# DredderGun/accbpg_and_fw

Hardware: AMD Instinct MI355X
Metric: D-opt iters/sec (m=2048,n=32768) (higher is better)
Workload: dtype f64; 1 GPU; D_opt_design(2048,32768) abpg_gain gamma=2 fp64, one independent instance per GPU; instances=1, instances_per_gpu=1, seeds=1..1, window=transient: iterations 5..161 from x0 = 1/n, linear_gram=False

## Files before the change

### accbpg_and_fw_amd/csrc/capi.hip

```cpp
#include <stdarg.h>
#include <string.h>
#include <stdlib.h>
#include <algorithm>

#include "internal.h"
#include "reduce.hpp"

namespace accbpg {

static thread_local char g_err[512] = "";

void set_last_error(const char* fmt, ...) {
    va_list ap;
    va_start(ap, fmt);
    vsnprintf(g_err, sizeof(g_err), fmt, ap);
    va_end(ap);
}

void note_tiles_fallback(const char* where) {
    static bool said = false;
    if (said) return;
    said = true;
    fprintf(stderr, "libaccbpg_hip: %s: the one-launch Cholesky abandoned a wait (another process on this GPU, or fewer "
                    "workgroups resident than the occupancy query promised); this handle factors with one launch per block "
// ... 462 lines not shown

extern "C" int accbpg_test_gemm(const double* A_dev, int64_t lda, const double* B_dev, int64_t ldb, double* C_dev,
                                int64_t ldc, int64_t M, int64_t N, int64_t K, int b_kmajor, double alpha,
                                double beta, int config, void* stream) {
    if (!A_dev || !B_dev || !C_dev || M <= 0 || N <= 0 || K <= 0) return ACCBPG_ERR_ARG;
    return launch_test_gemm(A_dev, lda, B_dev, ldb, C_dev, ldc, M, N, K, b_kmajor, alpha, beta, config,
                            (hipStream_t)stream);
}

extern "C" int accbpg_dopt_factor_in_small_launches(accbpg_dopt* h, int on) {
    if (!h || on < 0 || on > 2) return ACCBPG_ERR_ARG;
    const int64_t T = (h->m + NB - 1) / NB;
    value_forget(h);
    h->chol_tiles_off = on == 1 || (on == 2 && T * (T + 1) / 2 >= h->num_cu);
    return ACCBPG_OK;
}

extern "C" int accbpg_debug_plan_flags(int flags) {
    set_plan_flags(flags);
    return ACCBPG_OK;
}

extern "C" int accbpg_debug_chol_variant(accbpg_dopt* h, int bits) {
    if (!h) return ACCBPG_ERR_ARG;
    value_forget(h);
    h->chol_dbg = bits & 63;
    h->chol_tiles_off = (bits & 64) != 0;
    if (bits & 2048) h->chol_tiles_off = true;
    h->chol_stall_test = (bits & 128) ? 1 : 0;
    h->chol_spin_limit = (bits & 128) ? 200000 : 20000000;
    h->kern_variant = (bits >> 30) & 3;
    if (bits & 256) h->use_glds = false;
    if (bits & 512) h->use_glds = true;
    if (bits & 2048) {
        h->chol_two_level_T = (bits >> 12) & 0xfff;
        if ((bits >> 24) & 0x3f) h->chol_nk = (bits >> 24) & 0x3f;
    }
    return ACCBPG_OK;
}

extern "C" int accbpg_debug_chol_trace(accbpg_dopt* h, const double* gram_dev, int with_inverse, int64_t* stamps_host) {
    if (!h || !gram_dev || !stamps_host) return ACCBPG_ERR_ARG;
    if (!chol_tiles_usable(h)) {
        set_last_error("accbpg_debug_chol_trace: the one-launch Cholesky is not in use for this handle");
        return ACCBPG_ERR_ARG;
    }
    const int T = (int)((h->m + NB - 1) / NB);
    const size_t bytes = sizeof(long long) * (size_t)T * 32;
    if (!h->chol_trace) ACC_HIP(hipMalloc(&h->chol_trace, bytes));
    ACC_HIP(hipMemsetAsync(h->chol_trace, 0, bytes, h->stream));
    int rc = launch_cholesky(h, h->Lbuf, with_inverse ? h->Wbuf : nullptr, nullptr, gram_dev);
    if (rc == ACCBPG_OK) {
        hipError_t e = hipMemcpyAsync(stamps_host, h->chol_trace, bytes, hipMemcpyDeviceToHost, h->stream);
        if (e == hipSuccess) e = hipStreamSynchronize(h->stream);
        if (e != hipSuccess) rc = ACCBPG_ERR_HIP;
    }
    hipFree(h->chol_trace);
    h->chol_trace = nullptr;
    return rc;
}

extern "C" int accbpg_debug_gram_variant(accbpg_dopt* h, const double* x_dev, int variant, int iters, double* ms_host) {
    if (!h || !x_dev || !ms_host || iters <= 0) return ACCBPG_ERR_ARG;
    value_forget(h);
    return debug_gram_variant(h, x_dev, variant, iters, ms_host);
}
// ... 7 lines not shown
```

### accbpg_and_fw_amd/csrc/dopt_kernels.hip

```cpp
#include <mutex>
#include <unordered_map>
#include <type_traits>

#include "internal.h"
#include "mfma_tile.hpp"

namespace accbpg {

struct GramSeg {
    int64_t row0, col0, kb, ke;
    bool dual, whole;
};
constexpr int GRAM_RMAX = 4;
template <class T>
__device__ __forceinline__ GramSeg gram_segment(const TileRC* __restrict__ tiles, int64_t kiters, int64_t it,
                                                int64_t it1) {
    const int e = (int)(it / kiters);
    const int64_t off = it - (int64_t)e * kiters;
    const TileRC tr = tiles[e];
    GramSeg g;
    if (tr.d1 < 0) {
        g.row0 = (int64_t)tr.rb * T::BM; g.col0 = (int64_t)tr.cb * T::BN;
        g.kb = off; g.ke = min(kiters, off + (it1 - it));
        g.dual = false;
// ... 747 lines not shown
    }
    __syncthreads();
    for (int c = threadIdx.x; c < T::BN; c += NTHREADS) {
        double s = 0.0;
#pragma unroll
        for (int w = 0; w < T::WAVES_M; ++w) s += red[w * T::BN + c];
        if (col0 + c < n) out[col0 + c] = sign * s;
    }
}

template <class T, int CV = 0>
__device__ __forceinline__ void colnorm_glds_body(
    const double* __restrict__ W, int64_t ldw, const double* __restrict__ V, int64_t ldv, int64_t m, int64_t n,
    double* __restrict__ out, double sign) {
    if constexpr (CV == COLNORM_CV) colnorm_phases_body<T>(W, ldw, V, ldv, m, n, out, sign);
    else colnorm_restart_body<T, CV>(W, ldw, V, ldv, m, n, out, sign);
}

template <class T, int CV = 0>
__global__ __launch_bounds__(NTHREADS, 1) void colnorm_glds_kernel(
    const double* __restrict__ W, int64_t ldw, const double* __restrict__ V, int64_t ldv, int64_t m, int64_t n,
    double* __restrict__ out, double sign) {
    colnorm_glds_body<T, CV>(W, ldw, V, ldv, m, n, out, sign);
}
template <class T>
__global__ __launch_bounds__(NTHREADS, 1) void colnorm_glds_batch_kernel(
    const BatchInst* __restrict__ bt, BatchAct act, int64_t ldw, int64_t ldv, int64_t m, int64_t n,
    double* __restrict__ outbase, int64_t ldo, double sign) {
    const int inst = act.idx[blockIdx.y];
    const BatchInst bi = bt[inst];
    colnorm_glds_body<T, COLNORM_CV>(bi.Wbuf, ldw, bi.V, ldv, m, n, outbase + (int64_t)inst * ldo, sign);
}

template <class T>
__device__ __forceinline__ void gemm_ops_body(const GemmOp op) {
    extern __shared__ __attribute__((aligned(16))) double lds[];
    const int64_t row0 = (int64_t)blockIdx.y * T::BM, col0 = (int64_t)blockIdx.x * T::BN;
    if (row0 >= op.M || col0 >= op.N) return;
    if (op.lower_only && col0 > row0 + T::BM - 1) return;
    const bool va = ((reinterpret_cast<uintptr_t>(op.A) & 15) == 0) && ((op.lda & 1) == 0);
    const bool vb = ((reinterpret_cast<uintptr_t>(op.B) & 15) == 0) && ((op.ldb & 1) == 0);
    T t;
    t.zero();
    int64_t ksteps = (op.K + BK - 1) / BK;
    int64_t ks0 = 0;
    if (op.tri & 1) ks0 = max((int64_t)0, col0 - op.koff) / BK;
    if (op.tri & 2) ksteps = min(ksteps, max((int64_t)0, row0 + T::BM - op.koff + BK - 1) / BK);
    if (ks0 >= ksteps) {
        t.store_C(op.C, op.ldc, row0, col0, op.M, op.N, op.alpha, op.beta, op.lower_only != 0);
        return;
    }
    auto gload = [&](int64_t ks) {
        t.gload_A(op.A, op.lda, row0, op.M, ks * BK, op.K, va);
        if constexpr (T::BKM) t.gload_B_km(op.B, op.ldb, col0, op.N, ks * BK, op.K, vb);
        else t.gload_B_kc(op.B, op.ldb, col0, op.N, ks * BK, op.K, vb);
    };
    gload(ks0);
    t.sstore(lds);
    __syncthreads();
    int cur = 0;
    for (int64_t ks = ks0; ks < ksteps; ++ks) {
        const bool more = ks + 1 < ksteps;
        if (more) gload(ks + 1);
        t.compute(lds + cur * T::STAGE_ELEMS);
        if (more) t.sstore(lds + (cur ^ 1) * T::STAGE_ELEMS);
        __syncthreads();
        cur ^= 1;
    }
    t.store_C(op.C, op.ldc, row0, col0, op.M, op.N, op.alpha, op.beta, op.lower_only != 0);
}

template <class T>
__global__ __launch_bounds__(NTHREADS, 2) void gemm_ops_kernel(const GemmOp* __restrict__ ops) {
    gemm_ops_body<T>(ops[blockIdx.z]);
}
template <class T>
__global__ __launch_bounds__(NTHREADS, 2) void gemm_ops_batch_kernel(const GemmOp* __restrict__ ops, int per_inst, int begin,
                                                                    int count, BatchAct act) {
    const int a = blockIdx.z / count, o = blockIdx.z - a * count;
    gemm_ops_body<T>(ops[(int64_t)act.idx[a] * per_inst + begin + o]);
}

__device__ __forceinline__ void gemm_reduce_body(const RedOp r) {
    const int64_t total = (int64_t)r.M * r.N;
    const int64_t stride = (int64_t)gridDim.x * 256 * 2;
    for (int64_t e = 2 * ((int64_t)blockIdx.x * 256 + threadIdx.x); e < total; e += stride) {
        double2 acc = *reinterpret_cast<const double2*>(r.P + e);
        for (int p = 1; p < r.ns; ++p) {
            const double2 v = *reinterpret_cast<const double2*>(r.P + (int64_t)p * total + e);
            acc.x += v.x;
            acc.y += v.y;
        }
        const int64_t row = e / r.N, col = e - row * r.N;
        *reinterpret_cast<double2*>(r.C + row * r.ldc + col) = acc;
    }
}
__global__ __launch_bounds__(256) void gemm_reduce_kernel(const RedOp* __restrict__ reds) { gemm_reduce_body(reds[blockIdx.y]); }
__global__ __launch_bounds__(256) void gemm_reduce_batch_kernel(const RedOp* __restrict__ reds, int per_inst, int begin, int count,
                                                               BatchAct act) {
    const int a = blockIdx.y / count, o = blockIdx.y - a * count;
    gemm_reduce_body(reds[(int64_t)act.idx[a] * per_inst + begin + o]);
}

template <class T>
__global__ __launch_bounds__(NTHREADS, 1) void gemm_big_kernel(GemmOp op) {
    extern __shared__ __attribute__((aligned(16))) double lds[];
    const int64_t row0 = (int64_t)blockIdx.y * T::BM, col0 = (int64_t)blockIdx.x * T::BN;
    if (row0 >= op.M || col0 >= op.N) return;
    const bool va = ((reinterpret_cast<uintptr_t>(op.A) & 15) == 0) && ((op.lda & 1) == 0);
    const bool vb = ((reinterpret_cast<uintptr_t>(op.B) & 15) == 0) && ((op.ldb & 1) == 0);
    T t;
    t.zero();
    const int64_t ksteps = (op.K + BK - 1) / BK;
// ... 1404 lines not shown
    if (T <= CT_TMAX) {
        std::vector<CholJob> jobs;
        for (int d2 = 0; d2 < T; ++d2) jobs.push_back(CholJob{d2, d2});
        for (int j = 0; j < T; ++j)
            for (int i = j + 2; i < T; ++i) jobs.push_back(CholJob{i, j});
        ACC_TRY(set_lds(chol_tiles_kernel, CT_LDS_BYTES));
        int per_cu = 0;
        ACC_HIP(hipOccupancyMaxActiveBlocksPerMultiprocessor(&per_cu, chol_tiles_kernel, NTHREADS, CT_LDS_BYTES));
        h->chol_tiles_grid = (int)jobs.size();
        h->chol_slots = std::min(per_cu, 2) * h->num_cu;
        h->chol_tiles_ok = per_cu >= 1 && (int64_t)jobs.size() <= (int64_t)h->chol_slots;
        if (h->chol_tiles_ok) {
            ACC_HIP(hipMalloc(&h->chol_jobs, sizeof(CholJob) * jobs.size()));
            ACC_HIP(hipMemcpy(h->chol_jobs, jobs.data(), sizeof(CholJob) * jobs.size(), hipMemcpyHostToDevice));
            ACC_HIP(hipMalloc(&h->chol_ready, sizeof(int) * (size_t)(T * T + 5 * T)));
            ACC_HIP(hipMemset(h->chol_ready, 0, sizeof(int) * (size_t)(T * T + 5 * T)));
            ACC_HIP(hipMalloc(&h->chol_hand, sizeof(double) * (size_t)T * NB * NB));
            ACC_HIP(hipMalloc(&h->chol_aux, sizeof(double) * (size_t)T * CT_AUX));
            ACC_HIP(hipMalloc(&h->Gbuf, sizeof(double) * (size_t)m * m));
            ACC_HIP(hipMemset(h->Gbuf, 0, sizeof(double) * (size_t)m * m));
        }
    }

    ACC_TRY(set_lds(gram_streamk_kernel<TileBig<false, true>>, TileBig<false>::LDS_BYTES));
    ACC_TRY(set_lds(gram_streamk_kernel<TileBig<false, false>>, TileBig<false>::LDS_BYTES));
    ACC_TRY(set_lds(gram_streamk_kernel<TileSmall<false, true>>, TileSmall<false>::LDS_BYTES));
    ACC_TRY(set_lds(gram_streamk_kernel<TileSmall<false, false>>, TileSmall<false>::LDS_BYTES));
    ACC_TRY(set_lds(colnorm_kernel<TileBig<true, true>>, TileBig<true>::LDS_BYTES));
    ACC_TRY(set_lds(colnorm_kernel<TileBig<true, false>>, TileBig<true>::LDS_BYTES));
    ACC_TRY(set_lds(colnorm_kernel<TileSmall<true, true>>, TileSmall<true>::LDS_BYTES));
    ACC_TRY(set_lds(colnorm_kernel<TileSmall<true, false>>, TileSmall<true>::LDS_BYTES));
    ACC_TRY(set_lds(gemm_ops_kernel<TileSmall<true>>, TileSmall<true>::LDS_BYTES));
    ACC_TRY(set_lds(gemm_ops_kernel<TileSmall<false>>, TileSmall<false>::LDS_BYTES));
    ACC_TRY(set_lds(chol_step_kernel, CHOL_LDS_BYTES));
    ACC_TRY(set_lds(chol_syrk_kernel, SYRK_LDS_BYTES));
    ACC_TRY(set_lds(gemm_big_kernel<TileBig<true>>, TileBig<true>::LDS_BYTES));
    ACC_TRY(set_lds(gemm_big_kernel<TileBig<false>>, TileBig<false>::LDS_BYTES));
    return ACCBPG_OK;
}

template <class T>
static int gram_launch_t(accbpg_dopt* h, const double* x, double* gram) {
    if constexpr (!T::EDGE && T::BM == 256) {
        if (h->use_glds || h->has_duals) {
            const int64_t nc = h->gram_chunks > 1 ? h->gram_nc : h->n;
            for (int c = 0; c < h->gram_chunks; ++c) {
                const double* Vc = h->Vblk ? h->Vblk + (int64_t)c * h->m * nc : h->V + (int64_t)c * nc;
                const int64_t ldc = h->Vblk ? nc : h->ldv;
                const double* xc = x + (int64_t)c * nc;
                const double beta = c == 0 ? 0.0 : 1.0;
                const int all_slabs = h->gram_chunks > 1 ? 1 : 0;
                prof_begin(h, PROF_GRAM);
#define ACC_GRAM_ARGS Vc, ldc, h->m, nc, xc, h->tiles, h->wg_ranges, h->kiters, h->gram_nslot, h->slabs, gram, h->m, all_slabs
                if (h->kern_variant == 1)
                    ACC_LAUNCH_LDS((gram_streamk_glds_kernel<T, GRAM_GV ^ 128>), h->gram_grid, NTHREADS, T::G_LDS_BYTES, h->stream, ACC_GRAM_ARGS);
                else if (h->kern_variant == 3)
                    ACC_LAUNCH_LDS((gram_streamk_glds_kernel<T, 0>), h->gram_grid, NTHREADS, T::G_LDS_BYTES, h->stream, ACC_GRAM_ARGS);
                else if (h->kern_variant == 2)
                    ACC_LAUNCH_LDS((gram_streamk_glds_kernel<T, (GRAM_GV ^ 128) | 256>), h->gram_grid, NTHREADS, T::G_LDS_BYTES, h->stream, ACC_GRAM_ARGS);
                else
                    ACC_LAUNCH_LDS((gram_streamk_glds_kernel<T, GRAM_GV>), h->gram_grid, NTHREADS, T::G_LDS_BYTES, h->stream, ACC_GRAM_ARGS);
#undef ACC_GRAM_ARGS
                ACC_HIP(hipGetLastError());
                prof_end(h, PROF_GRAM);
                prof_begin(h, PROF_GRAMFIX);
                gram_fixup_kernel<T><<<h->ntiles * 2 * T::MI * FIX_PJ, NTHREADS, 0, h->stream>>>(
// ... 81 lines not shown
    bool xal = (reinterpret_cast<uintptr_t>(x) & 15) == 0;
    if (!xal && (h->has_duals || h->gram_chunks > 1)) {
        if (!h->xbuf) ACC_HIP(hipMalloc(&h->xbuf, sizeof(double) * (size_t)h->n));
        ACC_TRY(device_copy(h->xbuf, x, (size_t)h->n, h->stream));
        x = h->xbuf;
        xal = true;
    }
    if (h->big) {
        const bool interior = h->vec_ok && xal && (h->m % 256 == 0) && (h->n % BK == 0);
        if (interior) ACC_TRY((gram_launch_t<TileBig<false, false>>(h, x, gram)));
        else ACC_TRY((gram_launch_t<TileBig<false, true>>(h, x, gram)));
    } else {
        const bool interior = h->vec_ok && xal && (h->m % 64 == 0) && (h->n % BK == 0);
        if (interior) ACC_TRY((gram_launch_t<TileSmall<false, false>>(h, x, gram)));
        else ACC_TRY((gram_launch_t<TileSmall<false, true>>(h, x, gram)));
    }
    ACC_HIP(hipGetLastError());
    return ACCBPG_OK;
}

__global__ __launch_bounds__(256) void copy_kernel(double* __restrict__ dst, const double* __restrict__ src, size_t n) {
    const size_t stride = (size_t)gridDim.x * 256;
    for (size_t i = (size_t)blockIdx.x * 256 + threadIdx.x; i < n; i += stride) dst[i] = src[i];
}
int device_copy(double* dst, const double* src, size_t ndoubles, hipStream_t s) {
    if (ndoubles == 0 || dst == src) return ACCBPG_OK;
    size_t nb = (ndoubles + 255) / 256;
    if (nb > 4096) nb = 4096;
    copy_kernel<<<(unsigned)nb, 256, 0, s>>>(dst, src, ndoubles);
    ACC_HIP(hipGetLastError());
    return ACCBPG_OK;
}

int launch_gemm_ops(const GemmOp* ops_dev, int nops, int maxM, int maxN, bool b_kmajor, hipStream_t s) {
    if (nops <= 0 || maxM <= 0 || maxN <= 0) return ACCBPG_OK;
    dim3 grid((maxN + 63) / 64, (maxM + 63) / 64, nops);
    if (b_kmajor)
        gemm_ops_kernel<TileSmall<true>><<<grid, NTHREADS, TileSmall<true>::LDS_BYTES, s>>>(ops_dev);
    else
        gemm_ops_kernel<TileSmall<false>><<<grid, NTHREADS, TileSmall<false>::LDS_BYTES, s>>>(ops_dev);
    ACC_HIP(hipGetLastError());
    return ACCBPG_OK;
}

static std::mutex g_tiles_mu;
constexpr int TILES_RING = 16;
struct TilesRing {
    hipEvent_t ev[TILES_RING] = {};
    hipStream_t stream[TILES_RING] = {};
    int grid[TILES_RING] = {};
    long long issued = 0;
};
static TilesRing g_tiles[64];

bool chol_tiles_usable(const accbpg_dopt* h) {
    return h->chol_tiles_ok && !h->chol_tiles_off && (h->chol_dbg & 63) == 0;
}

static int launch_chol_tiles(accbpg_dopt* h, const double* src, double* A, double* Winv) {
    const int64_t m = h->m;
    const int T = (int)((m + NB - 1) / NB);
    CholInst ci;
    ci.src = src; ci.L = A; ci.Ldiag = h->Tbuf; ci.Winv = Winv; ci.logdet = h->dscal; ci.flags = h->dflag;
    ci.ready = h->chol_ready; ci.aux = h->chol_aux; ci.hand = h->chol_hand; ci.trace = h->chol_trace;
    const int dev = (h->device >= 0 && h->device < 64) ? h->device : 0;
    std::lock_guard<std::mutex> lk(g_tiles_mu);
    TilesRing& ring = g_tiles[dev];
    {
        int gmax = h->chol_tiles_grid;
        for (int i = 0; i < TILES_RING; ++i) gmax = std::max(gmax, ring.grid[i]);
        int together = std::max(1, h->chol_slots) / std::max(1, gmax);
// ... 34 lines not shown
        return ACCBPG_OK;
    }
    if (src != A) ACC_TRY(device_copy(A, src, (size_t)m * m, h->stream));
    const int nkp = (T >= h->chol_two_level_T) ? h->chol_nk : T;
    for (int k0 = 0; k0 < T; k0 += nkp) {
        const int kend = std::min(k0 + nkp, T) - 1;
        for (int kc = k0; kc <= kend; ++kc) {
            const int pend = (kc > k0) ? 1 : 0;
            const int npanel = T - kc;
            const int R = T - (kc + 1);
            int nupd = 0;
            if (pend) nupd = (kend >= T - 1) ? R * (R + 1) / 2 : R * (kend - kc);
            chol_step_kernel<<<npanel + nupd, NTHREADS, CHOL_LDS_BYTES, h->stream>>>(
                A, m, m, kc, pend, kend, T, h->dscal, h->dflag, h->chol_dbg, Winv, h->Tbuf);
        }
        const int Rr = T - (kend + 1);
        if (Rr > 0)
            chol_syrk_kernel<<<Rr * (Rr + 1) / 2, NTHREADS, SYRK_LDS_BYTES, h->stream>>>(A, m, m, k0, kend - k0 + 1, T);
    }
    h->diag_inv_ready = (Winv != nullptr);
    prof_end(h, PROF_CHOL);
    ACC_HIP(hipGetLastError());
    return ACCBPG_OK;
}

int launch_trtri(accbpg_dopt* h) {
    const int64_t m = h->m;
    const int T = (int)((m + NB - 1) / NB);
    prof_begin(h, PROF_TRTRI);
    if (!h->diag_inv_ready) trtri_diag_kernel<<<T, 64, 0, h->stream>>>(h->Tbuf, m, h->Wbuf, m, m);
    h->diag_inv_ready = false;
    for (const accbpg_dopt::MergeStage& st : h->merge_stages) {
        if (st.kind == 0) {
            ACC_TRY(launch_gemm_ops(h->ops + st.begin, st.end - st.begin, st.maxm, st.maxn, true, h->stream));
        } else {
            int gx = (int)std::min<int64_t>(1024, ((int64_t)st.maxm / 2 + 255) / 256);
            gemm_reduce_kernel<<<dim3(gx, st.end - st.begin), 256, 0, h->stream>>>(h->red + st.begin);
        }
    }
    prof_end(h, PROF_TRTRI);
    ACC_HIP(hipGetLastError());
    return ACCBPG_OK;
}

template <class T>
static void colnorm_launch_t(accbpg_dopt* h, const double* W, double* out, double sign, bool vw) {
    const int grid = (int)((h->n + T::BN - 1) / T::BN);
    colnorm_kernel<T><<<grid, NTHREADS, T::LDS_BYTES, h->stream>>>(W, h->m, h->V, h->ldv, h->m, h->n, out, sign, vw,
                                                                  h->vec_ok);
}

int launch_colnorm(accbpg_dopt* h, const double* W, double* out, double sign) {
    prof_begin(h, PROF_GRAD);
    const bool vw = ((reinterpret_cast<uintptr_t>(W) & 15) == 0) && ((h->m & 1) == 0);
    if (h->big) {
        const bool interior = vw && h->vec_ok && (h->m % 256 == 0) && (h->n % 128 == 0);
        if (interior && h->use_glds) {
            using T = TileBig<true, false>;
            const int grid = (int)(h->n / T::BN), lds = T::G_LDS_BYTES + 4 * T::BN * 8;
            if (h->kern_variant == 1)
                ACC_LAUNCH_LDS((colnorm_glds_kernel<T, COLNORM_CV ^ 256>), grid, NTHREADS, lds, h->stream, W, h->m, h->V, h->ldv, h->m, h->n, out, sign);
            else if (h->kern_variant == 2)
                ACC_LAUNCH_LDS((colnorm_glds_kernel<T, 96>), grid, NTHREADS, lds, h->stream, W, h->m, h->V, h->ldv, h->m, h->n, out, sign);
            else if (h->kern_variant == 3)
                ACC_LAUNCH_LDS((colnorm_glds_kernel<T, COLNORM_CV | 512>), grid, NTHREADS, lds, h->stream, W, h->m, h->V, h->ldv, h->m, h->n, out, sign);
            else
                ACC_LAUNCH_LDS((colnorm_glds_kernel<T, COLNORM_CV>), grid, NTHREADS, lds, h->stream, W, h->m, h->V, h->ldv, h->m, h->n, out, sign);
// ... 44 lines not shown
        for (int i = 0; i < TILES_RING; ++i) gmax = std::max(gmax, ring.grid[i]);
        int together = std::max(1, h0->chol_slots) / std::max(1, gmax);
        if (together > TILES_RING - 1) together = TILES_RING - 1;
        if (together < 1) together = 1;
        for (long long back = together; back <= TILES_RING && back <= ring.issued; ++back) {
            const int slot = (int)((ring.issued - back) % TILES_RING);
            if (ring.ev[slot] && ring.stream[slot] != b->stream) ACC_HIP(hipStreamWaitEvent(b->stream, ring.ev[slot], 0));
        }
    }
    chol_tiles_kernel<<<dim3(h0->chol_tiles_grid, act.n), NTHREADS, CT_LDS_BYTES, b->stream>>>(
        CholInst{}, b->chol_table[with_inverse ? 1 : 0], reinterpret_cast<const CholJob*>(h0->chol_jobs), m, m, T,
        h0->chol_spin_limit, 0, act);
    prof_end(h0, PROF_CHOL);
    ACC_HIP(hipGetLastError());
    {
        const int slot = (int)(ring.issued % TILES_RING);
        if (!ring.ev[slot]) ACC_HIP(hipEventCreateWithFlags(&ring.ev[slot], hipEventDisableTiming));
        ACC_HIP(hipEventRecord(ring.ev[slot], b->stream));
        ring.stream[slot] = b->stream;
        ring.grid[slot] = grid_all;
        ++ring.issued;
    }
    return ACCBPG_OK;
}

int launch_trtri_batch(accbpg_dopt_batch* b, const BatchAct& act) {
    accbpg_dopt* h0 = b->inst[0];
    prof_begin(h0, PROF_TRTRI);
    for (const accbpg_dopt::MergeStage& st : h0->merge_stages) {
        const int count = st.end - st.begin;
        if (count <= 0) continue;
        if (st.kind == 0) {
            dim3 grid((st.maxn + 63) / 64, (st.maxm + 63) / 64, count * act.n);
            gemm_ops_batch_kernel<TileSmall<true>><<<grid, NTHREADS, TileSmall<true>::LDS_BYTES, b->stream>>>(
                b->ops_all, b->ops_per_inst, st.begin, count, act);
        } else {
            int gx = (int)std::min<int64_t>(1024, ((int64_t)st.maxm / 2 + 255) / 256);
            gemm_reduce_batch_kernel<<<dim3(gx, count * act.n), 256, 0, b->stream>>>(b->red_all, b->red_per_inst, st.begin, count, act);
        }
    }
    prof_end(h0, PROF_TRTRI);
    ACC_HIP(hipGetLastError());
    return ACCBPG_OK;
}

int debug_grad_variant(accbpg_dopt* h, double* out, int var, int iters, double* ms_out) {
    using T = TileBig<true, false>;
    const bool vw = ((reinterpret_cast<uintptr_t>(h->Wbuf) & 15) == 0) && ((h->m & 1) == 0);
    if (!h->big || !h->use_glds || !vw || !h->vec_ok || h->m % 256 != 0 || h->n % 128 != 0) return ACCBPG_ERR_ARG;
    const int grid = (int)(h->n / T::BN), lds = T::G_LDS_BYTES + 4 * T::BN * 8;
    if (var != 0 && var != 3 && (var < 10 || var > 13)) return ACCBPG_ERR_ARG;
    hipEvent_t a, b;
    ACC_HIP(hipEventCreate(&a));
    if (hipEventCreate(&b) != hipSuccess) {
        hipEventDestroy(a);
        return ACCBPG_ERR_HIP;
    }
    auto launch = [&]() -> int {
#define ACC_LAUNCH_C(CC) \
    ACC_LAUNCH_LDS((colnorm_glds_kernel<T, CC>), grid, NTHREADS, lds, h->stream, h->Wbuf, h->m, h->V, h->ldv, h->m, h->n, out, -1.0)
        switch (var) {
            case 0: ACC_LAUNCH_C(COLNORM_CV); break;
            case 3: ACC_LAUNCH_C(COLNORM_CV | 512); break;
            case 10: ACC_LAUNCH_C(COLNORM_CV | 512 | 1); break;
            case 11: ACC_LAUNCH_C(COLNORM_CV | 512 | 2); break;
            case 12: ACC_LAUNCH_C(COLNORM_CV | 512 | 4); break;
            case 13: ACC_LAUNCH_C(COLNORM_CV | 512 | 8); break;
            default: return ACCBPG_ERR_ARG;
// ... 28 lines not shown
        lds_set = true;
    }
    prof_begin(h0, PROF_GRAD);
    colnorm_glds_batch_kernel<T><<<dim3((unsigned)(h0->n / T::BN), act.n), NTHREADS, T::G_LDS_BYTES + 4 * T::BN * 8, b->stream>>>(
        b->table, act, h0->m, h0->ldv, h0->m, h0->n, gbase, ldg, sign);
    prof_end(h0, PROF_GRAD);
    ACC_HIP(hipGetLastError());
    return ACCBPG_OK;
}

int launch_test_gemm(const double* A, int64_t lda, const double* B, int64_t ldb, double* C, int64_t ldc, int64_t M,
                     int64_t N, int64_t K, int b_kmajor, double alpha, double beta, int config, hipStream_t s) {
    GemmOp op{};
    op.A = A; op.B = B; op.C = C; op.lda = lda; op.ldb = ldb; op.ldc = ldc;
    op.M = (int)M; op.N = (int)N; op.K = (int)K; op.lower_only = 0; op.alpha = alpha; op.beta = beta;
    if (config == 1) {
        if (b_kmajor) {
            using T = TileBig<true>;
            ACC_TRY(set_lds(gemm_big_kernel<T>, T::LDS_BYTES));
            dim3 grid((unsigned)((N + T::BN - 1) / T::BN), (unsigned)((M + T::BM - 1) / T::BM));
            gemm_big_kernel<T><<<grid, NTHREADS, T::LDS_BYTES, s>>>(op);
        } else {
            using T = TileBig<false>;
            ACC_TRY(set_lds(gemm_big_kernel<T>, T::LDS_BYTES));
            dim3 grid((unsigned)((N + T::BN - 1) / T::BN), (unsigned)((M + T::BM - 1) / T::BM));
            gemm_big_kernel<T><<<grid, NTHREADS, T::LDS_BYTES, s>>>(op);
        }
    } else {
        GemmOp* d = nullptr;
        ACC_HIP(hipMalloc(&d, sizeof(GemmOp)));
        ACC_HIP(hipMemcpyAsync(d, &op, sizeof(GemmOp), hipMemcpyHostToDevice, s));
        ACC_TRY(set_lds(gemm_ops_kernel<TileSmall<true>>, TileSmall<true>::LDS_BYTES));
        ACC_TRY(set_lds(gemm_ops_kernel<TileSmall<false>>, TileSmall<false>::LDS_BYTES));
        int rc = launch_gemm_ops(d, 1, (int)M, (int)N, b_kmajor != 0, s);
        hipStreamSynchronize(s);
        hipFree(d);
        return rc;
    }
    ACC_HIP(hipGetLastError());
    return ACCBPG_OK;
}

int pipe_probe(int iters, int mode, double* ms_out, hipStream_t s) {
    int dev = 0;
    hipDeviceProp_t prop;
    ACC_HIP(hipGetDevice(&dev));
    ACC_HIP(hipGetDeviceProperties(&prop, dev));
    double* sink = nullptr;
    ACC_HIP(hipMalloc(&sink, 8));
    hipEvent_t a, b;
    ACC_HIP(hipEventCreate(&a));
    ACC_HIP(hipEventCreate(&b));
    pipe_probe_kernel<<<prop.multiProcessorCount, NTHREADS, 0, s>>>(iters / 10 + 1, mode, sink);
    ACC_HIP(hipEventRecord(a, s));
    pipe_probe_kernel<<<prop.multiProcessorCount, NTHREADS, 0, s>>>(iters, mode, sink);
    ACC_HIP(hipEventRecord(b, s));
    ACC_HIP(hipEventSynchronize(b));
    float ms = 0.f;
    ACC_HIP(hipEventElapsedTime(&ms, a, b));
    *ms_out = ms;
    hipEventDestroy(a); hipEventDestroy(b); hipFree(sink);
    return ACCBPG_OK;
}

int mfma_peak(int iters, double* tflops, hipStream_t s) {
    int dev = 0;
    hipDeviceProp_t prop;
// ... 25 lines not shown
```

### accbpg_and_fw_amd/csrc/internal.h

```cpp
#pragma once
#include <hip/hip_runtime.h>
#include <stdint.h>
#include <stdio.h>
#include <vector>

#include "../../include/accbpg_hip.h"

namespace accbpg {

void set_last_error(const char* fmt, ...);
void note_tiles_fallback(const char* where);

#define ACC_HIP(call)                                                                         \
    do {                                                                                      \
        hipError_t e__ = (call);                                                              \
        if (e__ != hipSuccess) {                                                              \
            ::accbpg::set_last_error("%s:%d: %s -> %s", __FILE__, __LINE__, #call,            \
                                     hipGetErrorString(e__));                                 \
            return ACCBPG_ERR_HIP;                                                            \
        }                                                                                     \
    } while (0)

#define ACC_TRY(call)                       \
    do {                                    \
// ... 162 lines not shown
    std::vector<accbpg::GemmOp> ops_host;
    std::vector<accbpg::RedOp> red_host;
    struct MergeStage { int kind, begin, end, maxm, maxn; };
    std::vector<MergeStage> merge_stages;
    accbpg::RedOp* red = nullptr;
    double* Pbuf = nullptr;
    accbpg::GemmOp* chol_op = nullptr;

    double *fw_x = nullptr, *fw_w = nullptr, *fw_H = nullptr, *fw_hv = nullptr;
    double* fw_hpin_dev = nullptr;
    bool fw_ready = false;
    struct FwSlot {
        accbpg_dopt* aux = nullptr;
        hipStream_t stream = nullptr;
        hipEvent_t ev_snap = nullptr;
        bool pending = false;
    };
    std::vector<FwSlot> fw_ring;
    int fw_ring_depth = 1;
    int fw_ring_small = 2;
    long long fw_ring_issued = 0, fw_ring_collected = 0;
    int fw_part_nblk = 0;
    bool fw_part_away = false;
    accbpg::FwRun* fw_run = nullptr;
    accbpg_fw_step* fw_steps_pin = nullptr;
    accbpg_fw_step* fw_steps_dev = nullptr;

    bool use_glds = true;
    int kern_variant = 0;
    bool diag_inv_ready = false;
    bool has_duals = false;
    int chol_nk = 8;
    int chol_two_level_T = 64;
    int chol_dbg = 0;
    bool chol_tiles_ok = false;
    bool chol_tiles_off = false;
    int chol_stall_test = 0;
    long long chol_spin_limit = 20000000;
    int chol_tiles_grid = 0;
    int chol_slots = 0;
    void* chol_jobs = nullptr;
    int* chol_ready = nullptr;
    double* chol_aux = nullptr;
    double* chol_hand = nullptr;
    long long* chol_trace = nullptr;
    double* Gbuf = nullptr;
    const double* last_x = nullptr;
    double* last_g = nullptr;
    int last_flag = 0;
    hipEvent_t ev_done = nullptr;
    bool val_reuse = true;
    bool val_valid = false;
    bool val_pending = false;
    bool val_hit = false;
    const double* val_x = nullptr;
    double* val_copy = nullptr;
    double val_f = 0.0;
    double val_answer = 0.0;
    int val_gen = 0;
    int64_t val_compares = 0, val_answered = 0;
    accbpg_dopt* val_peer = nullptr;
    std::vector<accbpg_dopt*> val_linked;
    bool prof_on = false;
    accbpg::ProfSlot prof[accbpg::PROF_COUNT];
};

// ... 16 lines not shown
    double* vpart = nullptr;
    double* vgg = nullptr;
    double* vws = nullptr;
    double* vpin = nullptr;
    accbpg::FwInst* fw_table = nullptr;
    accbpg::FwRunSlot* fw_runs = nullptr;
    accbpg_fw_step* fw_bsteps_pin = nullptr;
    accbpg_fw_step* fw_bsteps_dev = nullptr;
    accbpg::BatchAct pend_act;
    const double* pend_x = nullptr;
    double* pend_g = nullptr;
    int64_t pend_ldx = 0, pend_ldg = 0;
    int pend_flag = 0;
    bool pend_fused = false;
};
struct BatchVals { double v[accbpg::BATCH_MAX]; };

namespace accbpg {

int launch_gram_batch(accbpg_dopt_batch* b, const BatchAct& act, const double* xbase, int64_t ldx);
int launch_cholesky_batch(accbpg_dopt_batch* b, const BatchAct& act, bool with_inverse, const double* xbase, int64_t ldx);
int launch_trtri_batch(accbpg_dopt_batch* b, const BatchAct& act);
int launch_colnorm_batch(accbpg_dopt_batch* b, const BatchAct& act, double* gbase, int64_t ldg, double sign);

int dopt_init(accbpg_dopt* h);
int launch_gram(accbpg_dopt* h, const double* x, double* gram);
int launch_cholesky(accbpg_dopt* h, double* A , double* Winv = nullptr ,
                    const double* xcheck = nullptr ,
                    const double* src = nullptr ,
                    double* xkeep = nullptr );
bool chol_tiles_usable(const accbpg_dopt* h);
int launch_trtri(accbpg_dopt* h);
int launch_colnorm(accbpg_dopt* h, const double* W, double* out, double sign);
int launch_gemm_ops(const GemmOp* ops_dev, int nops, int maxM, int maxN, bool b_kmajor, hipStream_t s);
int launch_test_gemm(const double* A, int64_t lda, const double* B, int64_t ldb, double* C, int64_t ldc,
                     int64_t M, int64_t N, int64_t K, int b_kmajor, double alpha, double beta, int config,
                     hipStream_t s);
int build_plans(accbpg_dopt* h);
void set_plan_flags(int flags);
int debug_gram_variant(accbpg_dopt* h, const double* x, int var, int iters, double* ms_out);
int debug_grad_variant(accbpg_dopt* h, double* out, int var, int iters, double* ms_out);
int mfma_peak(int iters, double* tflops, hipStream_t s);
int pipe_probe(int iters, int mode, double* ms_out, hipStream_t s);

int64_t vec_ws_doubles(int64_t n);
int vec_scratch(double** pin, int** flags, double** out);

int vt_nsplit(int64_t m, int64_t n, int num_cu);
int launch_vt_times(const double* V, int64_t ldv, int64_t m, int64_t n, const double* q, double* upart, int nsplit,
                    double* u, bool vec_ok, hipStream_t s);
int launch_vt_times_batch(const KyInst* tab, int K, int64_t ldv, int64_t m, int64_t n, bool first, int nsplit,
                          hipStream_t s);
constexpr int VT_MAXSPLIT = 64;

int device_copy(double* dst, const double* src, size_t ndoubles, hipStream_t s);

void prof_begin(accbpg_dopt* h, ProfKind k);
void prof_end(accbpg_dopt* h, ProfKind k);

}
```

### accbpg_and_fw_amd/csrc/mfma_tile.hpp

```cpp
#pragma once
#include <hip/hip_runtime.h>
#include <stdint.h>
#include <type_traits>

namespace accbpg {

typedef double d4 __attribute__((ext_vector_type(4)));
typedef double d2 __attribute__((ext_vector_type(2)));

constexpr int BK = 16;
constexpr int SK = BK + 2;
constexpr int NTHREADS = 256;

__device__ __forceinline__ d2 load2_guard(const double* __restrict__ p, bool row_ok, int64_t k, int64_t K,
                                          bool vec_ok) {
    d2 v;
    if (row_ok && vec_ok && k + 1 < K) {
        v = *reinterpret_cast<const d2*>(p);
    } else {
        v.x = (row_ok && k < K) ? p[0] : 0.0;
        v.y = (row_ok && k + 1 < K) ? p[1] : 0.0;
    }
    return v;
}
// ... 91 lines not shown
        const int c = tid & 7, r = tid >> 3;
        const int64_t k = k0 + 2 * c;
        if constexpr (!EDGE) {
            const double* __restrict__ base = B + (col0 + r) * ldb + k;
#pragma unroll
            for (int p = 0; p < B_PASS; ++p) rb[p] = *reinterpret_cast<const d2*>(base + (int64_t)(32 * p) * ldb);
        } else {
#pragma unroll
            for (int p = 0; p < B_PASS; ++p) {
                const int64_t row = col0 + r + 32 * p;
                rb[p] = load2_guard(B + row * ldb + k, row < N, k, K, vec_ok);
            }
        }
    }
    __device__ __forceinline__ void gload_B_km(const double* __restrict__ B, int64_t ldb, int64_t col0, int64_t N,
                                               int64_t k0, int64_t K, bool vec_ok) {
        const int tid = threadIdx.x;
        const int c = 2 * (tid % BKM_TPR), r = tid / BKM_TPR;
        const int64_t col = col0 + c;
        if constexpr (!EDGE) {
            const double* __restrict__ base = B + (k0 + r) * ldb + col;
#pragma unroll
            for (int p = 0; p < B_PASS; ++p)
                rb[p] = *reinterpret_cast<const d2*>(base + (int64_t)(BKM_RPP * p) * ldb);
        } else {
#pragma unroll
            for (int p = 0; p < B_PASS; ++p) {
                const int64_t k = k0 + r + BKM_RPP * p;
                rb[p] = load2_guard(B + k * ldb + col, k < K, col, N, vec_ok);
            }
        }
    }

    __device__ __forceinline__ void sstore(double* __restrict__ stage) {
        const int tid = threadIdx.x;
        {
            const int c = tid & 7, r = tid >> 3;
#pragma unroll
            for (int p = 0; p < A_PASS; ++p)
                *reinterpret_cast<d2*>(stage + (r + 32 * p) * SK + 2 * c) = ra[p];
        }
        double* bs = stage + A_ELEMS;
        if constexpr (BKM) {
            const int c = 2 * (tid % BKM_TPR), r = tid / BKM_TPR;
#pragma unroll
            for (int p = 0; p < B_PASS; ++p)
                *reinterpret_cast<d2*>(bs + (r + BKM_RPP * p) * SBN + c) = rb[p];
        } else {
            const int c = tid & 7, r = tid >> 3;
#pragma unroll
            for (int p = 0; p < B_PASS; ++p)
                *reinterpret_cast<d2*>(bs + (r + 32 * p) * SK + 2 * c) = rb[p];
        }
    }

    double fa[2][MI], fb[2][NI];

    template <int SET>
    __device__ __forceinline__ void read_frag(const double* __restrict__ stage, int kk) {
        const int lane = threadIdx.x & 63, wave = __builtin_amdgcn_readfirstlane(threadIdx.x >> 6);
        const int wm = wave / WAVES_N, wn = wave % WAVES_N;
        const int lr = lane & 15, lq = lane >> 4;
        const double* as = stage + (16 * wm + lr) * SK + lq;
        const double* bs = stage + A_ELEMS + (BKM ? (lq * SBN + wn * WN + lr) : ((wn * WN + lr) * SK + lq));
#pragma unroll
        for (int i = 0; i < MI; ++i) fa[SET][i] = as[i * 16 * WAVES_M * SK + 4 * kk];
#pragma unroll
// ... 480 lines not shown
    }
    constexpr int REST = NMFMA - NDSR;
    constexpr int NV = NVALU > 0 ? (NVALU + 1) / 2 : 0;
#pragma unroll
    for (int i = 0; i < NV; ++i) {
        __builtin_amdgcn_sched_group_barrier(0x008, 1, 0);
        __builtin_amdgcn_sched_group_barrier(0x002, 2, 0);
    }
#pragma unroll
    for (int i = 0; i < NDSW; ++i) {
        __builtin_amdgcn_sched_group_barrier(0x008, 1, 0);
        __builtin_amdgcn_sched_group_barrier(0x200, 1, 0);
    }
    if (REST - NV - NDSW > 0) __builtin_amdgcn_sched_group_barrier(0x008, REST - NV - NDSW, 0);
}
template <int NMFMA, int NVMEM, int NDSR>
__device__ __forceinline__ void sched_post_barrier() {
#pragma unroll
    for (int i = 0; i < NVMEM; ++i) {
        __builtin_amdgcn_sched_group_barrier(0x008, 1, 0);
        __builtin_amdgcn_sched_group_barrier(0x020, 1, 0);
    }
#pragma unroll
    for (int i = 0; i < NDSR; ++i) {
        __builtin_amdgcn_sched_group_barrier(0x008, 1, 0);
        __builtin_amdgcn_sched_group_barrier(0x100, 1, 0);
    }
    __builtin_amdgcn_sched_group_barrier(0x008, NMFMA - NVMEM - NDSR, 0);
}

template <bool BKM, bool EDGE = true> using TileBig = Tile<256, 128, 64, 128, BKM, EDGE>;
template <bool BKM, bool EDGE = true> using TileSmall = Tile<64, 64, 32, 32, BKM, EDGE>;

}
```

Baseline: 63.31 iterations/s.

## Deepen merge GEMM global-load pipeline to three register stages with explicit vmcnt waits

Replaces the one-step-ahead global prefetch in the small-tile merge GEMM kernel with a register pipeline that keeps loads for up to three future K-steps in flight. It waits on the oldest batch with explicit s_waitcnt vmcnt and uses 32-bit offsets with masked zero-fill instead of guarded loads. Launch bounds are raised to 4 waves per SIMD to favour occupancy. This aims to hide global memory latency in the merge-stage GEMMs, at the cost of more registers per thread and scheduling risk. The old single-step path stays available behind a debug flag and is used when alignment or offset range conditions fail.

```diff
diff --git a/accbpg_and_fw_amd/csrc/capi.hip b/accbpg_and_fw_amd/csrc/capi.hip
--- a/accbpg_and_fw_amd/csrc/capi.hip
+++ b/accbpg_and_fw_amd/csrc/capi.hip
@@ -518,6 +518,7 @@
     h->kern_variant = (bits >> 30) & 3;
     if (bits & 256) h->use_glds = false;
     if (bits & 512) h->use_glds = true;
+    h->merge_one_step = (bits & 1024) != 0;
     if (bits & 2048) {
         h->chol_two_level_T = (bits >> 12) & 0xfff;
         if ((bits >> 24) & 0x3f) h->chol_nk = (bits >> 24) & 0x3f;
diff --git a/accbpg_and_fw_amd/csrc/dopt_kernels.hip b/accbpg_and_fw_amd/csrc/dopt_kernels.hip
--- a/accbpg_and_fw_amd/csrc/dopt_kernels.hip
+++ b/accbpg_and_fw_amd/csrc/dopt_kernels.hip
@@ -803,7 +803,52 @@
     colnorm_glds_body<T, COLNORM_CV>(bi.Wbuf, ldw, bi.V, ldv, m, n, outbase + (int64_t)inst * ldo, sign);
 }
 
-template <class T>
+constexpr int MERGE_DEPTH = 3;
+
+template <class T, int D>
+__device__ __forceinline__ void gemm_deep_loop(T& t, const GemmOp& op, int64_t row0, int64_t col0, int ks0, int ksteps,
+                                               double* __restrict__ lds) {
+    RegPipe<T, D> rp;
+    rp.setup(op, row0, col0);
+    const int last = ksteps - 1;
+    static_for<0, D>([&](auto jt) { rp.template issue<decltype(jt)::value>(min(ks0 + decltype(jt)::value, last)); });
+    rp.template wait_newest<D - 1>();
+    rp.template store<0>(lds, ks0);
+    __syncthreads();
+    int cur = 0;
+    int ks = ks0;
+    for (; ks + D < ksteps; ks += D) {
+        static_for<0, D>([&](auto jt) {
+            constexpr int j = decltype(jt)::value;
+            rp.template issue<j>(min(ks + j + D, last));
+            __builtin_amdgcn_sched_barrier(0);
+            t.compute(lds + cur * T::STAGE_ELEMS);
+            __builtin_amdgcn_sched_barrier(0);
+            rp.template wait_newest<D - 1>();
+            rp.template store<(j + 1) % D>(lds + (cur ^ 1) * T::STAGE_ELEMS, ks + j + 1);
+            __syncthreads();
+            __builtin_amdgcn_sched_barrier(0);
+            cur ^= 1;
+        });
+    }
+    static_for<0, D>([&](auto jt) {
+        constexpr int j = decltype(jt)::value;
+        const int s = ks + j;
+        if (s < ksteps) {
+            t.compute(lds + cur * T::STAGE_ELEMS);
+            if constexpr (j + 1 < D) {
+                if (s < last) {
+                    rp.template wait_newest<D - 2 - j>();
+                    rp.template store<j + 1>(lds + (cur ^ 1) * T::STAGE_ELEMS, s + 1);
+                }
+            }
+            __syncthreads();
+            cur ^= 1;
+        }
+    });
+}
+
+template <class T, int D = MERGE_DEPTH>
 __device__ __forceinline__ void gemm_ops_body(const GemmOp op) {
     extern __shared__ __attribute__((aligned(16))) double lds[];
     const int64_t row0 = (int64_t)blockIdx.y * T::BM, col0 = (int64_t)blockIdx.x * T::BN;
@@ -821,35 +866,41 @@
         t.store_C(op.C, op.ldc, row0, col0, op.M, op.N, op.alpha, op.beta, op.lower_only != 0);
         return;
     }
-    auto gload = [&](int64_t ks) {
-        t.gload_A(op.A, op.lda, row0, op.M, ks * BK, op.K, va);
-        if constexpr (T::BKM) t.gload_B_km(op.B, op.ldb, col0, op.N, ks * BK, op.K, vb);
-        else t.gload_B_kc(op.B, op.ldb, col0, op.N, ks * BK, op.K, vb);
-    };
-    gload(ks0);
-    t.sstore(lds);
-    __syncthreads();
-    int cur = 0;
-    for (int64_t ks = ks0; ks < ksteps; ++ks) {
-        const bool more = ks + 1 < ksteps;
-        if (more) gload(ks + 1);
-        t.compute(lds + cur * T::STAGE_ELEMS);
-        if (more) t.sstore(lds + (cur ^ 1) * T::STAGE_ELEMS);
+    bool deep = false;
+    if constexpr (D > 1) deep = RegPipe<T, D>::usable(op);
+    if (deep) {
+        if constexpr (D > 1) gemm_deep_loop<T, D>(t, op, row0, col0, (int)ks0, (int)ksteps, lds);
+    } else {
+        auto gload = [&](int64_t ks) {
+            t.gload_A(op.A, op.lda, row0, op.M, ks * BK, op.K, va);
+            if constexpr (T::BKM) t.gload_B_km(op.B, op.ldb, col0, op.N, ks * BK, op.K, vb);
+            else t.gload_B_kc(op.B, op.ldb, col0, op.N, ks * BK, op.K, vb);
+        };
+        gload(ks0);
+        t.sstore(lds);
         __syncthreads();
-        cur ^= 1;
+        int cur = 0;
+        for (int64_t ks = ks0; ks < ksteps; ++ks) {
+            const bool more = ks + 1 < ksteps;
+            if (more) gload(ks + 1);
+            t.compute(lds + cur * T::STAGE_ELEMS);
+            if (more) t.sstore(lds + (cur ^ 1) * T::STAGE_ELEMS);
+            __syncthreads();
+            cur ^= 1;
+        }
     }
     t.store_C(op.C, op.ldc, row0, col0, op.M, op.N, op.alpha, op.beta, op.lower_only != 0);
 }
 
-template <class T>
-__global__ __launch_bounds__(NTHREADS, 2) void gemm_ops_kernel(const GemmOp* __restrict__ ops) {
-    gemm_ops_body<T>(ops[blockIdx.z]);
-}
-template <class T>
-__global__ __launch_bounds__(NTHREADS, 2) void gemm_ops_batch_kernel(const GemmOp* __restrict__ ops, int per_inst, int begin,
+template <class T, int D = MERGE_DEPTH>
+__global__ __launch_bounds__(NTHREADS, D > 1 ? 4 : 2) void gemm_ops_kernel(const GemmOp* __restrict__ ops) {
+    gemm_ops_body<T, D>(ops[blockIdx.z]);
+}
+template <class T, int D = MERGE_DEPTH>
+__global__ __launch_bounds__(NTHREADS, D > 1 ? 4 : 2) void gemm_ops_batch_kernel(const GemmOp* __restrict__ ops, int per_inst, int begin,
                                                                     int count, BatchAct act) {
     const int a = blockIdx.z / count, o = blockIdx.z - a * count;
-    gemm_ops_body<T>(ops[(int64_t)act.idx[a] * per_inst + begin + o]);
+    gemm_ops_body<T, D>(ops[(int64_t)act.idx[a] * per_inst + begin + o]);
 }
 
 __device__ __forceinline__ void gemm_reduce_body(const RedOp r) {
@@ -2320,6 +2371,8 @@
     ACC_TRY(set_lds(colnorm_kernel<TileSmall<true, false>>, TileSmall<true>::LDS_BYTES));
     ACC_TRY(set_lds(gemm_ops_kernel<TileSmall<true>>, TileSmall<true>::LDS_BYTES));
     ACC_TRY(set_lds(gemm_ops_kernel<TileSmall<false>>, TileSmall<false>::LDS_BYTES));
+    ACC_TRY(set_lds(gemm_ops_kernel<TileSmall<true>, 1>, TileSmall<true>::LDS_BYTES));
+    ACC_TRY(set_lds(gemm_ops_kernel<TileSmall<false>, 1>, TileSmall<false>::LDS_BYTES));
     ACC_TRY(set_lds(chol_step_kernel, CHOL_LDS_BYTES));
     ACC_TRY(set_lds(chol_syrk_kernel, SYRK_LDS_BYTES));
     ACC_TRY(set_lds(gemm_big_kernel<TileBig<true>>, TileBig<true>::LDS_BYTES));
@@ -2467,11 +2520,15 @@
     return ACCBPG_OK;
 }
 
-int launch_gemm_ops(const GemmOp* ops_dev, int nops, int maxM, int maxN, bool b_kmajor, hipStream_t s) {
+int launch_gemm_ops(const GemmOp* ops_dev, int nops, int maxM, int maxN, bool b_kmajor, hipStream_t s, bool one_step) {
     if (nops <= 0 || maxM <= 0 || maxN <= 0) return ACCBPG_OK;
     dim3 grid((maxN + 63) / 64, (maxM + 63) / 64, nops);
-    if (b_kmajor)
+    if (b_kmajor && one_step)
+        gemm_ops_kernel<TileSmall<true>, 1><<<grid, NTHREADS, TileSmall<true>::LDS_BYTES, s>>>(ops_dev);
+    else if (b_kmajor)
         gemm_ops_kernel<TileSmall<true>><<<grid, NTHREADS, TileSmall<true>::LDS_BYTES, s>>>(ops_dev);
+    else if (one_step)
+        gemm_ops_kernel<TileSmall<false>, 1><<<grid, NTHREADS, TileSmall<false>::LDS_BYTES, s>>>(ops_dev);
     else
         gemm_ops_kernel<TileSmall<false>><<<grid, NTHREADS, TileSmall<false>::LDS_BYTES, s>>>(ops_dev);
     ACC_HIP(hipGetLastError());
@@ -2572,7 +2629,7 @@
     h->diag_inv_ready = false;
     for (const accbpg_dopt::MergeStage& st : h->merge_stages) {
         if (st.kind == 0) {
-            ACC_TRY(launch_gemm_ops(h->ops + st.begin, st.end - st.begin, st.maxm, st.maxn, true, h->stream));
+            ACC_TRY(launch_gemm_ops(h->ops + st.begin, st.end - st.begin, st.maxm, st.maxn, true, h->stream, h->merge_one_step));
         } else {
             int gx = (int)std::min<int64_t>(1024, ((int64_t)st.maxm / 2 + 255) / 256);
             gemm_reduce_kernel<<<dim3(gx, st.end - st.begin), 256, 0, h->stream>>>(h->red + st.begin);
@@ -2683,8 +2740,12 @@
         if (count <= 0) continue;
         if (st.kind == 0) {
             dim3 grid((st.maxn + 63) / 64, (st.maxm + 63) / 64, count * act.n);
-            gemm_ops_batch_kernel<TileSmall<true>><<<grid, NTHREADS, TileSmall<true>::LDS_BYTES, b->stream>>>(
-                b->ops_all, b->ops_per_inst, st.begin, count, act);
+            if (h0->merge_one_step)
+                gemm_ops_batch_kernel<TileSmall<true>, 1><<<grid, NTHREADS, TileSmall<true>::LDS_BYTES, b->stream>>>(
+                    b->ops_all, b->ops_per_inst, st.begin, count, act);
+            else
+                gemm_ops_batch_kernel<TileSmall<true>><<<grid, NTHREADS, TileSmall<true>::LDS_BYTES, b->stream>>>(
+                    b->ops_all, b->ops_per_inst, st.begin, count, act);
         } else {
             int gx = (int)std::min<int64_t>(1024, ((int64_t)st.maxm / 2 + 255) / 256);
             gemm_reduce_batch_kernel<<<dim3(gx, count * act.n), 256, 0, b->stream>>>(b->red_all, b->red_per_inst, st.begin, count, act);
@@ -2779,7 +2840,9 @@
         ACC_HIP(hipMemcpyAsync(d, &op, sizeof(GemmOp), hipMemcpyHostToDevice, s));
         ACC_TRY(set_lds(gemm_ops_kernel<TileSmall<true>>, TileSmall<true>::LDS_BYTES));
         ACC_TRY(set_lds(gemm_ops_kernel<TileSmall<false>>, TileSmall<false>::LDS_BYTES));
-        int rc = launch_gemm_ops(d, 1, (int)M, (int)N, b_kmajor != 0, s);
+        ACC_TRY(set_lds(gemm_ops_kernel<TileSmall<true>, 1>, TileSmall<true>::LDS_BYTES));
+        ACC_TRY(set_lds(gemm_ops_kernel<TileSmall<false>, 1>, TileSmall<false>::LDS_BYTES));
+        int rc = launch_gemm_ops(d, 1, (int)M, (int)N, b_kmajor != 0, s, config == 2);
         hipStreamSynchronize(s);
         hipFree(d);
         return rc;
diff --git a/accbpg_and_fw_amd/csrc/internal.h b/accbpg_and_fw_amd/csrc/internal.h
--- a/accbpg_and_fw_amd/csrc/internal.h
+++ b/accbpg_and_fw_amd/csrc/internal.h
@@ -218,6 +218,7 @@
     bool has_duals = false;
     int chol_nk = 8;
     int chol_two_level_T = 64;
+    bool merge_one_step = false;
     int chol_dbg = 0;
     bool chol_tiles_ok = false;
     bool chol_tiles_off = false;
@@ -300,7 +301,7 @@
 bool chol_tiles_usable(const accbpg_dopt* h);
 int launch_trtri(accbpg_dopt* h);
 int launch_colnorm(accbpg_dopt* h, const double* W, double* out, double sign);
-int launch_gemm_ops(const GemmOp* ops_dev, int nops, int maxM, int maxN, bool b_kmajor, hipStream_t s);
+int launch_gemm_ops(const GemmOp* ops_dev, int nops, int maxM, int maxN, bool b_kmajor, hipStream_t s, bool one_step = false);
 int launch_test_gemm(const double* A, int64_t lda, const double* B, int64_t ldb, double* C, int64_t ldc,
                      int64_t M, int64_t N, int64_t K, int b_kmajor, double alpha, double beta, int config,
                      hipStream_t s);
diff --git a/accbpg_and_fw_amd/csrc/mfma_tile.hpp b/accbpg_and_fw_amd/csrc/mfma_tile.hpp
--- a/accbpg_and_fw_amd/csrc/mfma_tile.hpp
+++ b/accbpg_and_fw_amd/csrc/mfma_tile.hpp
@@ -147,7 +147,9 @@
         }
     }
 
-    __device__ __forceinline__ void sstore(double* __restrict__ stage) {
+    __device__ __forceinline__ void sstore(double* __restrict__ stage) { sstore_regs(stage, ra, rb); }
+    static __device__ __forceinline__ void sstore_regs(double* __restrict__ stage, const d2 (&ra)[A_PASS],
+                                                       const d2 (&rb)[B_PASS]) {
         const int tid = threadIdx.x;
         {
             const int c = tid & 7, r = tid >> 3;
@@ -694,4 +696,102 @@
 template <bool BKM, bool EDGE = true> using TileBig = Tile<256, 128, 64, 128, BKM, EDGE>;
 template <bool BKM, bool EDGE = true> using TileSmall = Tile<64, 64, 32, 32, BKM, EDGE>;
 
+template <class T, int D>
+struct RegPipe {
+    static constexpr int LOADS = T::A_PASS + T::B_PASS;
+    static_assert(D >= 2 && (D - 1) * LOADS < 64, "vmcnt is a 6-bit counter");
+    typedef const __attribute__((address_space(1))) char* gptr;
+    typedef const __attribute__((address_space(1))) d2* gptr2;
+    d2 ra[D][T::A_PASS];
+    d2 rb[D][T::B_PASS];
+    gptr A, B;
+    int64_t ldb;
+    int K;
+    uint32_t oa[T::A_PASS];
+    uint32_t ob[T::B_PASS];
+    bool ina[T::A_PASS], inb[T::B_PASS];
+    int kl;
+
+    template <class Op>
+    static __device__ __forceinline__ bool usable(const Op& op) {
+        const int64_t span = (int64_t)1 << 29;
+        return ((reinterpret_cast<uintptr_t>(op.A) | reinterpret_cast<uintptr_t>(op.B)) & 15) == 0 &&
+               ((op.lda | op.ldb | op.K | (T::BKM ? op.N : 0)) & 1) == 0 && op.M * op.lda < span &&
+               (T::BKM ? op.K : op.N) * op.ldb < span;
+    }
+    template <class Op>
+    __device__ __forceinline__ void setup(const Op& op, int64_t row0, int64_t col0) {
+        const int tid = threadIdx.x;
+        A = (gptr)op.A;
+        B = (gptr)op.B;
+        ldb = op.ldb;
+        K = op.K;
+        const int r = tid >> 3;
+#pragma unroll
+        for (int p = 0; p < T::A_PASS; ++p) {
+            const int64_t row = row0 + r + 32 * p;
+            ina[p] = row < op.M;
+            oa[p] = (uint32_t)(((ina[p] ? row : 0) * op.lda + 2 * (tid & 7)) * 8);
+        }
+        if constexpr (T::BKM) {
+            const int64_t col = col0 + 2 * (tid % T::BKM_TPR);
+            kl = tid / T::BKM_TPR;
+#pragma unroll
+            for (int p = 0; p < T::B_PASS; ++p) {
+                inb[p] = col < op.N;
+                ob[p] = (uint32_t)(((kl + T::BKM_RPP * p) * op.ldb + (inb[p] ? col : 0)) * 8);
+            }
+        } else {
+            kl = 2 * (tid & 7);
+#pragma unroll
+            for (int p = 0; p < T::B_PASS; ++p) {
+                const int64_t row = col0 + r + 32 * p;
+                inb[p] = row < op.N;
+                ob[p] = (uint32_t)(((inb[p] ? row : 0) * op.ldb + kl) * 8);
+            }
+        }
+    }
+    static __device__ __forceinline__ d2 load(gptr base, uint32_t off, bool k_in) {
+        uint32_t o = k_in ? off : 0;
+        asm volatile("" : "+v"(o));
+        return *(gptr2)(base + o);
+    }
+    template <int S>
+    __device__ __forceinline__ void issue(int ks) {
+        const int k0 = ks * BK;
+        const bool kin = k0 + 2 * (int)(threadIdx.x & 7) < K;
+        const gptr a0 = A + (int64_t)k0 * 8;
+#pragma unroll
+        for (int p = 0; p < T::A_PASS; ++p) ra[S][p] = load(a0, oa[p], kin);
+        if constexpr (T::BKM) {
+            const gptr b0 = B + (int64_t)k0 * ldb * 8;
+#pragma unroll
+            for (int p = 0; p < T::B_PASS; ++p) rb[S][p] = load(b0, ob[p], k0 + kl + T::BKM_RPP * p < K);
+        } else {
+            const gptr b0 = B + (int64_t)k0 * 8;
+#pragma unroll
+            for (int p = 0; p < T::B_PASS; ++p) rb[S][p] = load(b0, ob[p], kin);
+        }
+    }
+    template <int NEWEST>
+    static __device__ __forceinline__ void wait_newest() {
+        asm volatile("s_waitcnt vmcnt(%0)" ::"n"(NEWEST * LOADS) : "memory");
+    }
+    template <int S>
+    __device__ __forceinline__ void store(double* __restrict__ stage, int ks) {
+        const int k0 = ks * BK;
+        const bool kin = k0 + 2 * (int)(threadIdx.x & 7) < K;
+        const d2 zero = d2{0.0, 0.0};
+#pragma unroll
+        for (int p = 0; p < T::A_PASS; ++p)
+            if (!(ina[p] && kin)) ra[S][p] = zero;
+#pragma unroll
+        for (int p = 0; p < T::B_PASS; ++p) {
+            const bool in = T::BKM ? (inb[p] && k0 + kl + T::BKM_RPP * p < K) : (inb[p] && kin);
+            if (!in) rb[S][p] = zero;
+        }
+        T::sstore_regs(stage, ra[S], rb[S]);
+    }
+};
+
 }
```

New measurement: 63.84 iterations/s, median of 6. No clear change (+0.8%).
